# waicool20/BoofCV

Measured on AMD Instinct MI355X. Metric: 1080p frames/sec detect+describe+associate, higher is better.
Workload: dtype f32 detect / f64 describe / associate: fp16 MFMA candidate filter + exact fp64 re-score; 1 GPU; batch of 256 1920x1080 GrayF32 per GPU: Fast-Hessian detect + SURF-64 (stable) describe + greedy L2 associate with the next frame; batch_per_gpu=256, width=1920, height=1080, ranks_seen=1

## Files before the change

boofcv_amd/csrc/hessian.hip:

```cpp
#include "hessian_dev.h"

struct HessParams {
	ImgView ii;
	int skip, w, h, nlevels;
	int nrun, runLevel[BHIP_MAX_LEVELS];
	float* out;
	long long levelStride, imageStrideOut;
	int outStride;
	HessLevel lv[BHIP_MAX_LEVELS];
	HessLevelSource from[BHIP_MAX_LEVELS];
	int srcBorder[BHIP_MAX_LEVELS];
	int srcW, srcH;
};

template <class T>
__global__ __launch_bounds__(256) void k_hessian(HessParams P) {
	const int x = blockIdx.x * blockDim.x + threadIdx.x;
	const int y = blockIdx.y;
	const int img = blockIdx.z / P.nrun;
	const int level = P.runLevel[blockIdx.z - img * P.nrun];
	if (x >= P.w) return;
	const HessLevel L = P.lv[level];
	if (P.from[level].src) {
		const bool inner = x >= L.border && x < P.w - L.border && y >= L.border && y < P.h - L.border;
		const int bp = P.srcBorder[level];
		const int px = 2 * x, py = 2 * y;
		const bool srcInner = px >= bp && px < P.srcW - bp && py >= bp && py < P.srcH - bp;
		if (srcInner == inner) {
			const HessLevelSource S = P.from[level];
			if (S.inPlace) return;
			P.out[(long long)img * P.imageStrideOut + (long long)level * P.levelStride + (long long)y * P.outStride + x] =
				S.src[(long long)img * S.imageStride + (long long)(y * S.step) * S.stride + x * S.step];
			return;
		}
	}
	const T* __restrict__ d = (const T*)P.ii.data + (long long)img * P.ii.imageStride;
	P.out[(long long)img * P.imageStrideOut + (long long)level * P.levelStride + (long long)y * P.outStride + x] =
		hessianCompute<T>(d, P.ii.stride, P.ii.width, P.ii.height, L, P.skip, P.w, P.h, x, y);
}

template <class T>
int bhip_launch_hessian(bhip_ctx* ctx, DevImg<const T> ii, int skip, int nlevels, const int* sizes, DevImg<float> level0, long long levelStride,
						const HessLevelSource* from, unsigned int skipMask) {
	if (nlevels > BHIP_MAX_LEVELS) return bhip_fail(ctx, BHIP_ERR_UNSUPPORTED, "too many scales per octave");
	const int batch = ii.batch;
	HessParams P;
	P.ii = bhip_kernel_view(ii);
	P.skip = skip;
	P.w = ii.width / skip;
	P.h = ii.height / skip;
	P.nlevels = nlevels;
	P.out = level0.data; P.levelStride = levelStride; P.imageStrideOut = level0.imageStride; P.outStride = level0.stride;
	for (int i = 0; i < nlevels; i++) {
		P.lv[i] = bhipMakeHessLevel(sizes[i], skip);
		P.from[i] = from ? from[i] : HessLevelSource{nullptr, 0, 0, 1, 0};
		P.srcBorder[i] = 0;
		if (P.from[i].src) {
			if (skip % 2 != 0) return bhip_fail(ctx, BHIP_ERR_INVALID, "a shared level needs an octave at half the step");
			P.srcBorder[i] = bhipMakeHessLevel(sizes[i], skip / 2).border;
		}
	}
	P.srcW = skip >= 2 ? ii.width / (skip / 2) : 0;
	P.srcH = skip >= 2 ? ii.height / (skip / 2) : 0;
	P.nrun = 0;
	for (int i = 0; i < nlevels; i++)
		if (!(skipMask & (1u << i))) P.runLevel[P.nrun++] = i;
	if (P.w <= 0 || P.h <= 0 || P.nrun == 0) return BHIP_OK;
	dim3 grid((P.w + 255) / 256, P.h, batch * P.nrun);
	{
		const double bytes = 4.0 * ii.width * ii.height * batch + 4.0 * P.nrun * (double)P.w * P.h * batch;
		ProfScope ps(ctx, skip == 1 ? "k_hessian_skip1" : "k_hessian_skipN", bytes);
		hipLaunchKernelGGL(k_hessian<T>, grid, dim3(256), 0, ctx->stream, P);
	}
	BHIP_HIP(ctx, hipGetLastError());
	return BHIP_OK;
}
template int bhip_launch_hessian(bhip_ctx*, DevImg<const int32_t>, int, int, const int*, DevImg<float>, long long, const HessLevelSource*, unsigned int);
template int bhip_launch_hessian(bhip_ctx*, DevImg<const float>, int, int, const int*, DevImg<float>, long long, const HessLevelSource*, unsigned int);
```

boofcv_amd/csrc/hessian_dev.h:

```cpp
#pragma once
#include "common.h"

struct HessLevel {
	int size;
	int bS, bL, rF, rS;
	int border, lost;
	float norm;
	int r1, r2, r3, b;
};

template <class T>
__device__ __forceinline__ T block_zero(const T* __restrict__ d, int stride, int W, int H, int x0, int y0, int x1, int y1) {
	x0 = min(x0, W - 1);
	y0 = min(y0, H - 1);
	x1 = min(x1, W - 1);
	y1 = min(y1, H - 1);
	const int cx0 = max(x0, 0), cy0 = max(y0, 0), cx1 = max(x1, 0), cy1 = max(y1, 0);
	const T vbr = d[(long long)cy1 * stride + cx1], vtr = d[(long long)cy0 * stride + cx1];
	const T vbl = d[(long long)cy1 * stride + cx0], vtl = d[(long long)cy0 * stride + cx0];
	const T br = (x1 >= 0 && y1 >= 0) ? vbr : T(0);
	const T tr = (y0 >= 0 && x1 >= 0) ? vtr : T(0);
	const T bl = (x0 >= 0 && y1 >= 0) ? vbl : T(0);
	const T tl = (x0 >= 0 && y0 >= 0) ? vtl : T(0);
	return br - tr - bl + tl;
}

template <class T>
__device__ __forceinline__ float hessianCompute(const T* __restrict__ d, int stride, int W, int H, const HessLevel& L, int skip, int w, int h, int x, int y) {
	const bool inner = x >= L.border && x < w - L.border && y >= L.border && y < h - L.border;
	const int xx = x * skip, yy = y * skip;
	float Dxx, Dyy, Dxy;
	if (inner) {
		const int col = L.lost + (x - L.border) * skip;
		const long long top = (long long)(yy - L.rS - 1) * stride + col;
		const long long bot = top + (long long)L.bL * stride;
		const int bS = L.bS;
		Dxx = (float)(d[bot + 3 * bS] - d[top + 3 * bS] - d[bot] + d[top]);
		Dxx -= (float)(T(3) * (d[bot + 2 * bS] - d[top + 2 * bS] - d[bot + bS] + d[top + bS]));

		const long long l = (long long)(yy - L.rF - 1) * stride + (L.rF - L.rS) + col;
		const long long r = l + L.bL;
		const long long ro1 = (long long)bS * stride;
		Dyy = (float)(d[r + 3 * ro1] - d[l + 3 * ro1] - d[r] + d[l]);
		Dyy -= (float)(T(3) * (d[r + 2 * ro1] - d[l + 2 * ro1] - d[r + ro1] + d[l + ro1]));

		const long long y1 = (long long)(yy - bS - 1) * stride + (L.rF - bS) + col;
		const long long y2 = y1 + ro1;
		const long long y3 = y2 + stride;
		const long long y4 = y3 + ro1;
		const int x3 = bS + 1, x4 = x3 + bS;
		Dxy = (float)(d[y2 + bS] - d[y1 + bS] - d[y2] + d[y1]);
		Dxy -= (float)(d[y2 + x4] - d[y1 + x4] - d[y2 + x3] + d[y1 + x3]);
		Dxy += (float)(d[y4 + x4] - d[y3 + x4] - d[y4 + x3] + d[y3 + x3]);
		Dxy -= (float)(d[y4 + bS] - d[y3 + bS] - d[y4] + d[y3]);
	} else {
		T ret = 0;
		ret += block_zero<T>(d, stride, W, H, xx - L.r2 - 1, yy - L.r3 - 1, xx + L.r2, yy + L.r3) * T(1);
		ret += block_zero<T>(d, stride, W, H, xx - L.r1 - 1, yy - L.r3 - 1, xx + L.r1, yy + L.r3) * T(-3);
		Dxx = (float)ret;
		ret = 0;
		ret += block_zero<T>(d, stride, W, H, xx - L.r3 - 1, yy - L.r2 - 1, xx + L.r3, yy + L.r2) * T(1);
		ret += block_zero<T>(d, stride, W, H, xx - L.r3 - 1, yy - L.r1 - 1, xx + L.r3, yy + L.r1) * T(-3);
		Dyy = (float)ret;
		ret = 0;
		const int b = L.b;
		ret += block_zero<T>(d, stride, W, H, xx - b - 1, yy - b - 1, xx - 1, yy - 1) * T(1);
		ret += block_zero<T>(d, stride, W, H, xx, yy - b - 1, xx + b, yy - 1) * T(-1);
		ret += block_zero<T>(d, stride, W, H, xx, yy, xx + b, yy + b) * T(1);
		ret += block_zero<T>(d, stride, W, H, xx - b - 1, yy, xx - 1, yy + b) * T(-1);
		Dxy = (float)ret;
	}
	Dxx *= L.norm;
	Dxy *= L.norm;
	Dyy *= L.norm;
	return Dxx * Dyy - 0.81f * Dxy * Dxy;
}

static inline HessLevel bhipMakeHessLevel(int size, int skip) {
	HessLevel L;
	L.size = size;
	L.bS = size / 3;
	L.bL = size - L.bS - 1;
	L.rF = size / 2;
	L.rS = L.bL / 2;
	const int borderOrig = L.rF + 1 + (skip - (L.rF + 1) % skip);
	L.border = borderOrig / skip;
	L.lost = borderOrig - L.rF - 1;
	L.norm = 1.0f / (float)(size * size);
	const int blockW = size / 3, blockH = size - blockW - 1;
	L.r1 = blockW / 2;
	L.r2 = blockW + L.r1;
	L.r3 = blockH / 2;
	L.b = size / 3;
	return L;
}
```

Measured before the change: 14120 frames/s.

## Stage Hessian integral-image taps in LDS with vectorized row loads for large skips

For octaves with power-of-two skip of at least 4, the Hessian kernel is split into a border/frame kernel and a row-tiled interior kernel. The interior kernel loads the ten tap rows per output row with 2- or 4-word vector loads into LDS, grouped by residue modulo skip, and then evaluates the box-filter taps from LDS. This replaces strided scattered global gathers, and blocks are interleaved across 8 images. The cost is an extra kernel launch, host-side planning, and more complex indexing, with a fallback to the old gather path when the layout does not fit.

```diff
diff --git a/boofcv_amd/csrc/hessian.hip b/boofcv_amd/csrc/hessian.hip
--- a/boofcv_amd/csrc/hessian.hip
+++ b/boofcv_amd/csrc/hessian.hip
@@ -1,4 +1,5 @@
 #include "hessian_dev.h"
+#include <algorithm>
 
 struct HessParams {
 	ImgView ii;
@@ -14,12 +15,7 @@
 };
 
 template <class T>
-__global__ __launch_bounds__(256) void k_hessian(HessParams P) {
-	const int x = blockIdx.x * blockDim.x + threadIdx.x;
-	const int y = blockIdx.y;
-	const int img = blockIdx.z / P.nrun;
-	const int level = P.runLevel[blockIdx.z - img * P.nrun];
-	if (x >= P.w) return;
+__device__ __forceinline__ void hessianPixel(const HessParams& P, int img, int level, int x, int y) {
 	const HessLevel L = P.lv[level];
 	if (P.from[level].src) {
 		const bool inner = x >= L.border && x < P.w - L.border && y >= L.border && y < P.h - L.border;
@@ -37,6 +33,211 @@
 	const T* __restrict__ d = (const T*)P.ii.data + (long long)img * P.ii.imageStride;
 	P.out[(long long)img * P.imageStrideOut + (long long)level * P.levelStride + (long long)y * P.outStride + x] =
 		hessianCompute<T>(d, P.ii.stride, P.ii.width, P.ii.height, L, P.skip, P.w, P.h, x, y);
+}
+
+template <class T>
+__global__ __launch_bounds__(256) void k_hessian(HessParams P) {
+	const int x = blockIdx.x * blockDim.x + threadIdx.x;
+	const int y = blockIdx.y;
+	const int img = blockIdx.z / P.nrun;
+	const int level = P.runLevel[blockIdx.z - img * P.nrun];
+	if (x >= P.w) return;
+	hessianPixel<T>(P, img, level, x, y);
+}
+
+#define BHIP_HESS_ROWS 10
+__host__ __device__ constexpr int hessRowWords(int r) { return r >= 2 && r < 6 ? 2 : 4; }
+
+struct HessFrame {
+	int x0, x1, y0, y1;
+	int count;
+};
+struct HessFrameParams {
+	HessFrame fr[BHIP_MAX_LEVELS];
+};
+
+template <class T>
+__global__ __launch_bounds__(256) void k_hessian_frame(HessParams P, HessFrameParams F) {
+	const int img = blockIdx.y / P.nrun;
+	const int run = blockIdx.y - img * P.nrun;
+	const HessFrame f = F.fr[run];
+	int idx = blockIdx.x * blockDim.x + threadIdx.x;
+	if (idx >= f.count) return;
+	const int above = f.y0 * P.w, below = (P.h - f.y1) * P.w;
+	int x, y;
+	if (idx < above + below) {
+		y = idx / P.w;
+		x = idx - y * P.w;
+		if (idx >= above) y += f.y1 - f.y0;
+	} else {
+		idx -= above + below;
+		const int side = P.w - (f.x1 - f.x0);
+		y = idx / side;
+		x = idx - y * side;
+		y += f.y0;
+		if (x >= f.x0) x += f.x1 - f.x0;
+	}
+	hessianPixel<T>(P, img, P.runLevel[run], x, y);
+}
+
+struct HessRowLevel {
+	int level;
+	int x0, nx, y0, ny;
+	int TX, ntiles, G;
+	float norm;
+	int dy[BHIP_HESS_ROWS], dc[BHIP_HESS_ROWS], base[BHIP_HESS_ROWS];
+	int tap[32];
+};
+struct HessRowParams {
+	ImgView ii;
+	int skip, batch, nlv;
+	int ymin, nrows;
+	int tilesPerRow;
+	int blocksPerImage;
+	float* out;
+	long long levelStride, imageStrideOut;
+	int outStride;
+	HessRowLevel lv[BHIP_MAX_LEVELS];
+};
+
+template <class T>
+struct HessTapsLds {
+	const T* lds;
+	const int* tap;
+	__device__ __forceinline__ T xx(int r, int k) const { return lds[tap[4 * r + k]]; }
+	__device__ __forceinline__ T yy(int k, int s) const { return lds[tap[8 + 2 * k + s]]; }
+	__device__ __forceinline__ T xy(int r, int c) const { return lds[tap[16 + 4 * r + c]]; }
+};
+
+typedef unsigned int hess_u2 __attribute__((ext_vector_type(2), aligned(4)));
+typedef unsigned int hess_u4 __attribute__((ext_vector_type(4), aligned(4)));
+
+template <class T>
+__global__ __launch_bounds__(256) void k_hessian_rows(HessRowParams P) {
+	extern __shared__ __attribute__((aligned(16))) unsigned int hessLds[];
+	const int slot = blockIdx.x >> 3;
+	const int img = (slot / P.blocksPerImage) * 8 + (blockIdx.x & 7);
+	if (img >= P.batch) return;
+	const int within = slot % P.blocksPerImage;
+	const int y = P.ymin + within / P.tilesPerRow;
+	int tile = within % P.tilesPerRow, li = 0;
+	while (li < P.nlv - 1 && tile >= P.lv[li].ntiles) { tile -= P.lv[li].ntiles; li++; }
+	const HessRowLevel& L = P.lv[li];
+	if (y < L.y0 || y >= L.y0 + L.ny) return;
+	const int first = tile * L.TX;
+	const int n = min(L.TX, L.nx - first);
+	const int W = P.ii.width;
+	const unsigned int* __restrict__ d = (const unsigned int*)P.ii.data + (long long)img * P.ii.imageStride;
+
+	const int q = threadIdx.x;
+	if (q < n + L.G - L.TX) {
+		unsigned int v[BHIP_HESS_ROWS][4];
+#pragma unroll
+		for (int r = 0; r < BHIP_HESS_ROWS; r++) {
+			const int rw = hessRowWords(r);
+			const int Y = y * P.skip + L.dy[r];
+			const int c = first * P.skip + L.dc[r] + P.skip * q;
+			const unsigned int* __restrict__ src = d + (long long)Y * P.ii.stride + c;
+			if (c >= 0 && c + rw <= W) {
+				if (rw == 4) { const hess_u4 t = *(const hess_u4*)src; v[r][0] = t.x; v[r][1] = t.y; v[r][2] = t.z; v[r][3] = t.w; }
+				else { const hess_u2 t = *(const hess_u2*)src; v[r][0] = t.x; v[r][1] = t.y; }
+			} else {
+#pragma unroll
+				for (int e = 0; e < rw; e++) v[r][e] = c + e >= 0 && c + e < W ? src[e] : 0;
+			}
+		}
+#pragma unroll
+		for (int r = 0; r < BHIP_HESS_ROWS; r++) {
+			unsigned int* dst = hessLds + L.base[r] + q;
+#pragma unroll
+			for (int e = 0; e < hessRowWords(r); e++) dst[e * L.G] = v[r][e];
+		}
+	}
+	__syncthreads();
+
+	const int i = threadIdx.x;
+	if (i >= n) return;
+	float Dxx, Dyy, Dxy;
+	hessianInnerExpr<T>(HessTapsLds<T>{(const T*)hessLds + i, L.tap}, Dxx, Dyy, Dxy);
+	P.out[(long long)img * P.imageStrideOut + (long long)L.level * P.levelStride + (long long)y * P.outStride + L.x0 + first + i] =
+		hessianDeterminant(Dxx, Dyy, Dxy, L.norm);
+}
+
+static bool hessPlanRows(const HessParams& P, int batch, HessRowParams& R, HessFrameParams& F, int* ldsBytes) {
+	const int skip = P.skip;
+	if (skip < 4 || (skip & (skip - 1)) != 0) return false;
+	R.ii = P.ii; R.skip = skip; R.batch = batch; R.nlv = 0;
+	R.out = P.out; R.levelStride = P.levelStride; R.imageStrideOut = P.imageStrideOut; R.outStride = P.outStride;
+	R.tilesPerRow = 0;
+	int ymin = P.h, ymax = 0, ldsWords = 0;
+	for (int run = 0; run < P.nrun; run++) {
+		const int level = P.runLevel[run];
+		const HessLevel& L = P.lv[level];
+		HessFrame& f = F.fr[run];
+		f = HessFrame{0, 0, 0, 0, P.w * P.h};
+		int x0 = L.border, x1 = P.w - L.border, y0 = L.border, y1 = P.h - L.border;
+		const HessLevelSource& S = P.from[level];
+		if (S.src) {
+			if (!S.inPlace) continue;
+			const int bp = P.srcBorder[level];
+			x0 = std::max(x0, (bp + 1) / 2); x1 = std::min(x1, (P.srcW - bp + 1) / 2);
+			y0 = std::max(y0, (bp + 1) / 2); y1 = std::min(y1, (P.srcH - bp + 1) / 2);
+		}
+		if (x1 <= x0 || y1 <= y0) continue;
+		if (S.src) {
+			f = HessFrame{x0, x1, y0, y1, P.w * P.h - (x1 - x0) * (y1 - y0)};
+			continue;
+		}
+		HessRowLevel& V = R.lv[R.nlv];
+		V.level = level; V.x0 = x0; V.nx = x1 - x0; V.y0 = y0; V.ny = y1 - y0; V.norm = L.norm;
+		int off[BHIP_HESS_ROWS][4], nt[BHIP_HESS_ROWS];
+		for (int r = 0; r < 2; r++) {
+			V.dy[r] = -L.rS - 1 + r * L.bL; nt[r] = 4;
+			for (int k = 0; k < 4; k++) off[r][k] = k * L.bS;
+		}
+		for (int k = 0; k < 4; k++) {
+			V.dy[2 + k] = -L.rF - 1 + k * L.bS; nt[2 + k] = 2;
+			for (int s = 0; s < 2; s++) off[2 + k][s] = L.rF - L.rS + s * L.bL;
+		}
+		for (int r = 0; r < 4; r++) {
+			V.dy[6 + r] = -L.bS - 1 + hessXyOffset(r, L.bS); nt[6 + r] = 4;
+			for (int c = 0; c < 4; c++) off[6 + r][c] = L.rF - L.bS + hessXyOffset(c, L.bS);
+		}
+		int plane[BHIP_HESS_ROWS][4], grp[BHIP_HESS_ROWS][4], maxGroup = 0;
+		bool ok = true;
+		for (int r = 0; r < BHIP_HESS_ROWS; r++) {
+			V.dc[r] = L.lost + off[r][0];
+			for (int k = 0; k < nt[r]; k++) {
+				const int rel = off[r][k] - off[r][0];
+				plane[r][k] = rel % skip;
+				grp[r][k] = rel / skip;
+				maxGroup = std::max(maxGroup, grp[r][k]);
+				if (plane[r][k] >= hessRowWords(r)) ok = false;
+			}
+		}
+		const int txCap = 256 - (maxGroup + 1);
+		if (!ok || txCap < 64) return false;
+		V.ntiles = (V.nx + txCap - 1) / txCap;
+		V.TX = (V.nx + V.ntiles - 1) / V.ntiles;
+		V.G = V.TX + maxGroup + 1;
+		int words = 0;
+		for (int r = 0; r < BHIP_HESS_ROWS; r++) { V.base[r] = words; words += hessRowWords(r) * V.G; }
+		for (int j = 0; j < 32; j++) {
+			const int r = j < 8 ? j / 4 : j < 16 ? 2 + (j - 8) / 2 : 6 + (j - 16) / 4;
+			const int k = j < 8 ? j % 4 : j < 16 ? (j - 8) % 2 : (j - 16) % 4;
+			V.tap[j] = V.base[r] + plane[r][k] * V.G + grp[r][k];
+		}
+		ldsWords = std::max(ldsWords, words);
+		f = HessFrame{x0, x1, y0, y1, P.w * P.h - (x1 - x0) * (y1 - y0)};
+		ymin = std::min(ymin, y0); ymax = std::max(ymax, y1);
+		R.tilesPerRow += V.ntiles;
+		R.nlv++;
+	}
+	if (R.nlv == 0) return false;
+	R.ymin = ymin; R.nrows = ymax - ymin;
+	R.blocksPerImage = R.nrows * R.tilesPerRow;
+	*ldsBytes = ldsWords * 4;
+	return true;
 }
 
 template <class T>
@@ -66,11 +267,23 @@
 	for (int i = 0; i < nlevels; i++)
 		if (!(skipMask & (1u << i))) P.runLevel[P.nrun++] = i;
 	if (P.w <= 0 || P.h <= 0 || P.nrun == 0) return BHIP_OK;
-	dim3 grid((P.w + 255) / 256, P.h, batch * P.nrun);
-	{
-		const double bytes = 4.0 * ii.width * ii.height * batch + 4.0 * P.nrun * (double)P.w * P.h * batch;
+	const double bytes = 4.0 * ii.width * ii.height * batch + 4.0 * P.nrun * (double)P.w * P.h * batch;
+	HessRowParams R;
+	HessFrameParams F;
+	int ldsBytes = 0;
+	if (bhip_env_flag("BHIP_DETECT_GATHER") || !hessPlanRows(P, batch, R, F, &ldsBytes)) {
+		dim3 grid((P.w + 255) / 256, P.h, batch * P.nrun);
 		ProfScope ps(ctx, skip == 1 ? "k_hessian_skip1" : "k_hessian_skipN", bytes);
 		hipLaunchKernelGGL(k_hessian<T>, grid, dim3(256), 0, ctx->stream, P);
+	} else {
+		int maxCount = 0;
+		for (int i = 0; i < P.nrun; i++) maxCount = std::max(maxCount, F.fr[i].count);
+		if (maxCount > 0) {
+			ProfScope ps(ctx, "k_hessian_frame");
+			hipLaunchKernelGGL(k_hessian_frame<T>, dim3((maxCount + 255) / 256, batch * P.nrun), dim3(256), 0, ctx->stream, P, F);
+		}
+		ProfScope ps(ctx, "k_hessian_rows", bytes);
+		hipLaunchKernelGGL(k_hessian_rows<T>, dim3(8 * ((batch + 7) / 8) * R.blocksPerImage), dim3(256), ldsBytes, ctx->stream, R);
 	}
 	BHIP_HIP(ctx, hipGetLastError());
 	return BHIP_OK;
diff --git a/boofcv_amd/csrc/hessian_dev.h b/boofcv_amd/csrc/hessian_dev.h
--- a/boofcv_amd/csrc/hessian_dev.h
+++ b/boofcv_amd/csrc/hessian_dev.h
@@ -25,6 +25,42 @@
 	return br - tr - bl + tl;
 }
 
+template <class T, class Taps>
+__device__ __forceinline__ void hessianInnerExpr(const Taps& t, float& Dxx, float& Dyy, float& Dxy) {
+	Dxx = (float)(t.xx(1, 3) - t.xx(0, 3) - t.xx(1, 0) + t.xx(0, 0));
+	Dxx -= (float)(T(3) * (t.xx(1, 2) - t.xx(0, 2) - t.xx(1, 1) + t.xx(0, 1)));
+
+	Dyy = (float)(t.yy(3, 1) - t.yy(3, 0) - t.yy(0, 1) + t.yy(0, 0));
+	Dyy -= (float)(T(3) * (t.yy(2, 1) - t.yy(2, 0) - t.yy(1, 1) + t.yy(1, 0)));
+
+	Dxy = (float)(t.xy(1, 1) - t.xy(0, 1) - t.xy(1, 0) + t.xy(0, 0));
+	Dxy -= (float)(t.xy(1, 3) - t.xy(0, 3) - t.xy(1, 2) + t.xy(0, 2));
+	Dxy += (float)(t.xy(3, 3) - t.xy(2, 3) - t.xy(3, 2) + t.xy(2, 2));
+	Dxy -= (float)(t.xy(3, 1) - t.xy(2, 1) - t.xy(3, 0) + t.xy(2, 0));
+}
+
+__device__ __forceinline__ float hessianDeterminant(float Dxx, float Dyy, float Dxy, float norm) {
+	Dxx *= norm;
+	Dxy *= norm;
+	Dyy *= norm;
+	return Dxx * Dyy - 0.81f * Dxy * Dxy;
+}
+
+__host__ __device__ __forceinline__ int hessXyOffset(int i, int bS) { return i == 0 ? 0 : i == 1 ? bS : i == 2 ? bS + 1 : 2 * bS + 1; }
+
+template <class T>
+struct HessTapsGlobal {
+	const T* __restrict__ d;
+	long long top, l, y1, stride;
+	int bS, bL;
+	__device__ __forceinline__ HessTapsGlobal(const T* __restrict__ d_, int stride_, const HessLevel& L, int yy, int col)
+		: d(d_), top((long long)(yy - L.rS - 1) * stride_ + col), l((long long)(yy - L.rF - 1) * stride_ + (L.rF - L.rS) + col),
+		  y1((long long)(yy - L.bS - 1) * stride_ + (L.rF - L.bS) + col), stride(stride_), bS(L.bS), bL(L.bL) {}
+	__device__ __forceinline__ T xx(int r, int k) const { return d[top + (long long)(r * bL) * stride + k * bS]; }
+	__device__ __forceinline__ T yy(int k, int s) const { return d[l + (long long)(k * bS) * stride + s * bL]; }
+	__device__ __forceinline__ T xy(int r, int c) const { return d[y1 + (long long)hessXyOffset(r, bS) * stride + hessXyOffset(c, bS)]; }
+};
+
 template <class T>
 __device__ __forceinline__ float hessianCompute(const T* __restrict__ d, int stride, int W, int H, const HessLevel& L, int skip, int w, int h, int x, int y) {
 	const bool inner = x >= L.border && x < w - L.border && y >= L.border && y < h - L.border;
@@ -32,27 +68,7 @@
 	float Dxx, Dyy, Dxy;
 	if (inner) {
 		const int col = L.lost + (x - L.border) * skip;
-		const long long top = (long long)(yy - L.rS - 1) * stride + col;
-		const long long bot = top + (long long)L.bL * stride;
-		const int bS = L.bS;
-		Dxx = (float)(d[bot + 3 * bS] - d[top + 3 * bS] - d[bot] + d[top]);
-		Dxx -= (float)(T(3) * (d[bot + 2 * bS] - d[top + 2 * bS] - d[bot + bS] + d[top + bS]));
-
-		const long long l = (long long)(yy - L.rF - 1) * stride + (L.rF - L.rS) + col;
-		const long long r = l + L.bL;
-		const long long ro1 = (long long)bS * stride;
-		Dyy = (float)(d[r + 3 * ro1] - d[l + 3 * ro1] - d[r] + d[l]);
-		Dyy -= (float)(T(3) * (d[r + 2 * ro1] - d[l + 2 * ro1] - d[r + ro1] + d[l + ro1]));
-
-		const long long y1 = (long long)(yy - bS - 1) * stride + (L.rF - bS) + col;
-		const long long y2 = y1 + ro1;
-		const long long y3 = y2 + stride;
-		const long long y4 = y3 + ro1;
-		const int x3 = bS + 1, x4 = x3 + bS;
-		Dxy = (float)(d[y2 + bS] - d[y1 + bS] - d[y2] + d[y1]);
-		Dxy -= (float)(d[y2 + x4] - d[y1 + x4] - d[y2 + x3] + d[y1 + x3]);
-		Dxy += (float)(d[y4 + x4] - d[y3 + x4] - d[y4 + x3] + d[y3 + x3]);
-		Dxy -= (float)(d[y4 + bS] - d[y3 + bS] - d[y4] + d[y3]);
+		hessianInnerExpr<T>(HessTapsGlobal<T>(d, stride, L, yy, col), Dxx, Dyy, Dxy);
 	} else {
 		T ret = 0;
 		ret += block_zero<T>(d, stride, W, H, xx - L.r2 - 1, yy - L.r3 - 1, xx + L.r2, yy + L.r3) * T(1);
@@ -70,10 +86,7 @@
 		ret += block_zero<T>(d, stride, W, H, xx - b - 1, yy, xx - 1, yy + b) * T(-1);
 		Dxy = (float)ret;
 	}
-	Dxx *= L.norm;
-	Dxy *= L.norm;
-	Dyy *= L.norm;
-	return Dxx * Dyy - 0.81f * Dxy * Dxy;
+	return hessianDeterminant(Dxx, Dyy, Dxy, L.norm);
 }
 
 static inline HessLevel bhipMakeHessLevel(int size, int skip) {
```

Result: faster. 14430 frames/s (median of 6 runs) (+2.2%).
